# yjh0410/YOLO-Nano

Measured on NVIDIA B200. Metric: images/sec YOLO-Nano-1.0x 416 bs256 fp32-parity e2e (backbone+neck+head+decode+NMS), higher is better.
Workload: dtype f32 (tcgen05 3xTF32 split, fp32 accumulate)

## Files before the change

### yolo_nano_b200/csrc/common.cuh

```cuda
#pragma once
#include <cuda_bf16.h>
#include <cuda_runtime.h>
#include <stdint.h>
#include <limits.h>
#include <stdlib.h>

#include "yolonano_b200.h"

namespace ynb {

constexpr int kNumSMs = 148;

__device__ __forceinline__ float apply_act(float v, int act) {
  if (act == YNB_ACT_RELU) return fmaxf(v, 0.0f);
  if (act == YNB_ACT_LEAKY) return v > 0.0f ? v : 0.1f * v;
  return v;
}

__device__ __forceinline__ float softmax_exp(float d) { return __expf(d); }
__device__ __forceinline__ float class_score(float sum, float obj) { return __fmul_rn(__fdiv_rn(1.0f, sum), obj); }

struct ChanMap {
  int gap_at;
  int gap;
  __host__ __device__ __forceinline__ int slot(int j) const { return j + (j >= gap_at ? gap : 0); }
};
__host__ __device__ inline ChanMap dense_map() { return ChanMap{INT_MAX, 0}; }

// ... 14 lines not shown
  *reinterpret_cast<uint2*>(p) = make_uint2(pack_bf16x2(v.x, v.y), pack_bf16x2(v.z, v.w));
}
__device__ __forceinline__ float to_float(float v) { return v; }
__device__ __forceinline__ float to_float(bf16 v) { return __bfloat162float(v); }

inline int round_up(int v, int m) { return (v + m - 1) / m * m; }
inline int64_t round_up64(int64_t v, int64_t m) { return (v + m - 1) / m * m; }

struct LaunchCounter {
  int64_t n = 0;
};
extern thread_local LaunchCounter* g_counter;

__device__ __forceinline__ void pdl_trigger() { asm volatile("griddepcontrol.launch_dependents;" ::: "memory"); }
__device__ __forceinline__ void pdl_wait() { asm volatile("griddepcontrol.wait;" ::: "memory"); }

inline bool pdl_enabled() {
  static int v = -1;
  if (v < 0) v = getenv("YNB_NO_PDL") ? 0 : 1;
  return v == 1;
}

template <typename... KArgs, typename... Args>
inline cudaError_t launch_pdl(void (*kern)(KArgs...), dim3 grid, dim3 block, size_t smem, cudaStream_t st,
                              Args&&... args) {
  cudaLaunchConfig_t cfg{};
  cfg.gridDim = grid;
  cfg.blockDim = block;
  cfg.dynamicSmemBytes = smem;
  cfg.stream = st;
  cudaLaunchAttribute attr[1];
  attr[0].id = cudaLaunchAttributeProgrammaticStreamSerialization;
  attr[0].val.programmaticStreamSerializationAllowed = 1;
  cfg.attrs = attr;
  cfg.numAttrs = pdl_enabled() ? 1 : 0;
  return cudaLaunchKernelEx(&cfg, kern, static_cast<KArgs>(args)...);
}

#define YNB_COUNT_LAUNCH()                  \
  do {                                      \
    if (::ynb::g_counter) ::ynb::g_counter->n++; \
  } while (0)

}
```

### yolo_nano_b200/csrc/gemm_tc.cuh

```cuda
#pragma once
#include <cuda.h>

#include <cstring>

#include "common.cuh"
#include "ptx_sm100.cuh"

namespace ynb {

constexpr int kTcThreads = 512;
constexpr int kTcSplitWarp0 = 8, kTcProducerWarp = 12, kTcMmaWarp = 13;
constexpr int kTcProducers = 3;
constexpr int kTcBM = 128;
constexpr int kTcBK = 32;
constexpr int kTcAStageBytes = kTcBM * 128;
constexpr int kTcMaxStages = 8;
constexpr int kTcSmemBudget = 232448;
constexpr int kTcMaxMain = 4;

struct TcGemmParams {
  int num_steps;
  int chunks_per_tap;
  int is3x3;
  int mode;
  int bf16_in;
  int out_bf16;
  int num_stages;
  int w_resident;
  int64_t M;
  int64_t num_tiles;
  int H, W, TH, TW, tiles_x, tiles_y;
  int N, Npad;
  int nmain;
  int nacc;
  int merge_corr;
  int ksub;
  int presplit;
  int a2_step;
  int stack_b;
  int acc_stages;
  uint32_t tmem_cols;
  uint32_t a_box_bytes;
  float* out;
  int out_ld, out_off, out_step;
  ChanMap omap;
  const float* bias;
  int act;
  const float* pass;
  int pass_ld;
  int tma_store;
  struct Decode {
// ... 61 lines not shown
  const int box_alo = p.presplit ? 1 : -1;
  const int box_whi = p.w_resident ? -1 : 1 + (p.presplit ? 1 : 0);
  const int box_wlo = (p.w_resident || !split) ? -1 : box_whi + 1;
  const int nboxes = 1 + (box_alo >= 0) + (box_whi >= 0) + (box_wlo >= 0);
  const int nprod = nboxes < kTcProducers ? nboxes : kTcProducers;
  const TcSmemLayout lay = tc_smem_layout(p.Npad, p.num_steps, p.num_stages, p.w_resident != 0, split);
  const uint32_t w_chunk_bytes = lay.w_chunk_bytes;
  const uint32_t a_bytes = kTcAStageBytes * (split ? 2 : 1);
  const uint32_t stage_bytes = lay.stage_bytes;
  const uint32_t w_res_bytes = lay.bias_off - lay.w_res_off;
  float* s_bias = reinterpret_cast<float*>(smem + lay.bias_off);
  uint64_t* bars = reinterpret_cast<uint64_t*>(smem + lay.bar_off);
  uint64_t* full = bars;
  uint64_t* ready = bars + kTcMaxStages;
  uint64_t* empty = bars + 2 * kTcMaxStages;
  uint64_t* tmem_full = bars + 3 * kTcMaxStages;
  uint64_t* tmem_empty = bars + 3 * kTcMaxStages + 2;
  uint64_t* w_full = bars + 3 * kTcMaxStages + 4;
  uint32_t* tmem_ptr = reinterpret_cast<uint32_t*>(bars + 3 * kTcMaxStages + 5);

  const int warp = threadIdx.x >> 5, lane = threadIdx.x & 31;
  pdl_trigger();

  if (warp == kTcProducerWarp && lane == 0) {
    ptx::prefetch_tmap(&tmA);
    if (p.presplit || p.a2_step > 0) ptx::prefetch_tmap(&tmAlo);
    ptx::prefetch_tmap(&tmWhi);
    if (split) ptx::prefetch_tmap(&tmWlo);
    if (p.tma_store) ptx::prefetch_tmap(&tmOut);
    for (int s = 0; s < p.num_stages; ++s) {
      ptx::mbar_init(&full[s], nprod);
      ptx::mbar_init(&ready[s], 4);
      ptx::mbar_init(&empty[s], 1);
    }
    for (int a = 0; a < 2; ++a) {
      ptx::mbar_init(&tmem_full[a], 1);
      ptx::mbar_init(&tmem_empty[a], 4);
    }
    ptx::mbar_init(w_full, 1);
    ptx::fence_barrier_init();
  }
  if (warp == kTcMmaWarp) {
    ptx::tmem_alloc(tmem_ptr, p.tmem_cols);
    ptx::tmem_relinquish();
  }
  if (warp < 4) {
    for (int i = threadIdx.x; i < p.Npad; i += 128) s_bias[i] = i < p.N ? __ldg(p.bias + i) : 0.0f;
  }
  ptx::tc_fence_before_sync();
  __syncthreads();
  ptx::tc_fence_after_sync();
  const uint32_t tmem_base = *tmem_ptr;

  auto stage_a = [&](int s) { return smem + (size_t)s * stage_bytes; };
  auto stage_alo = [&](int s) { return smem + (size_t)s * stage_bytes + kTcAStageBytes; };
  auto w_hi_ptr = [&](int s, int step) {
    return p.w_resident ? smem + lay.w_res_off + (size_t)step * w_chunk_bytes * (split ? 2 : 1)
                        : smem + (size_t)s * stage_bytes + a_bytes;
  };
  auto w_lo_ptr = [&](int s, int step) { return w_hi_ptr(s, step) + w_chunk_bytes; };

  const int acc_cols = p.Npad * p.nacc;
  const uint32_t step_tx = p.a_box_bytes * (p.presplit ? 2 : 1) + (p.w_resident ? 0 : w_chunk_bytes * (split ? 2 : 1));
  const bool splitters_on = split && !p.presplit;

  if (warp == kTcProducerWarp && p.w_resident && ptx::elect_one()) {
    ptx::mbar_arrive_expect_tx(w_full, w_res_bytes);
    for (int st = 0; st < p.num_steps; ++st) {
      ptx::tma_load_2d(w_hi_ptr(0, st), &tmWhi, w_full, st * kchunk, 0);
      if (split) ptx::tma_load_2d(w_lo_ptr(0, st), &tmWlo, w_full, st * kchunk, 0);
    }
  }
  pdl_wait();

  const int prole = warp == kTcProducerWarp ? 0 : (warp == 14 ? 1 : (warp == 15 ? 2 : -1));
  if (prole >= 0) {
    if (prole < nprod && ptx::elect_one()) {
      const bool do_a = 0 % nprod == prole;
      const bool do_alo = box_alo >= 0 && box_alo % nprod == prole;
      const bool do_whi = box_whi >= 0 && box_whi % nprod == prole;
      const bool do_wlo = box_wlo >= 0 && box_wlo % nprod == prole;
      const uint32_t my_tx = (do_a ? p.a_box_bytes : 0u) + (do_alo ? p.a_box_bytes : 0u) +
                             (do_whi ? w_chunk_bytes : 0u) + (do_wlo ? w_chunk_bytes : 0u);
      int s = 0;
      uint32_t ph = 0;
      bool ok = true;
      for (int64_t tile = blockIdx.x; tile < p.num_tiles && ok; tile += gridDim.x) {
        int b = 0, y0 = 0, x0 = 0;
        if (p.is3x3) {
          int per_img = p.tiles_x * p.tiles_y;
          b = (int)(tile / per_img);
          int r = (int)(tile - (int64_t)b * per_img);
          y0 = (r / p.tiles_x) * p.TH;
          x0 = (r % p.tiles_x) * p.TW;
        }
        for (int st = 0; st < p.num_steps; ++st) {
          ok = ptx::mbar_wait(&empty[s], ph ^ 1, p.err_flag, 1);
          if (!ok) break;
          ptx::mbar_arrive_expect_tx(&full[s], my_tx);
          if (p.is3x3) {
            int tap = st / p.chunks_per_tap, kc = st - tap * p.chunks_per_tap;
            int dy = tap / 3, dx = tap - dy * 3;
            if (do_a) ptx::tma_load_4d(stage_a(s), &tmA, &full[s], kc * kchunk, x0 + dx - 1, y0 + dy - 1, b);
            if (do_alo) ptx::tma_load_4d(stage_alo(s), &tmAlo, &full[s], kc * kchunk, x0 + dx - 1, y0 + dy - 1, b);
          } else {
            if (do_a) {
              const bool second = p.a2_step > 0 && st >= p.a2_step;
              ptx::tma_load_2d(stage_a(s), second ? &tmAlo : &tmA, &full[s], (second ? st - p.a2_step : st) * kchunk,
                               (int)(tile * kTcBM));
            }
          }
          if (do_whi) ptx::tma_load_2d(w_hi_ptr(s, st), &tmWhi, &full[s], st * kchunk, 0);
          if (do_wlo) ptx::tma_load_2d(w_lo_ptr(s, st), &tmWlo, &full[s], st * kchunk, 0);
          if (prole == 0) YNB_TRACE(1, tile, st);
          if (++s == p.num_stages) { s = 0; ph ^= 1; }
        }
      }
    }
  } else if (warp == kTcMmaWarp) {
    if (ptx::elect_one()) {
      const uint32_t idesc = ptx::make_idesc(2 , kTcBM, p.Npad);
      const uint32_t idesc2 = ptx::make_idesc(2, kTcBM, 2 * p.Npad);
      const uint32_t idesc_bf = ptx::make_idesc(1 , kTcBM, p.Npad);
      int s = 0;
      uint32_t ph = 0;
      int acc = 0;
      uint32_t acc_ph = 0;
      bool ok = true;
      if (p.w_resident) ok = ptx::mbar_wait(w_full, 0, p.err_flag, 2);
      for (int64_t tile = blockIdx.x; tile < p.num_tiles && ok; tile += gridDim.x) {
        ok = ptx::mbar_wait(&tmem_empty[acc], acc_ph ^ 1, p.err_flag, 3);
        if (!ok) break;
        ptx::tc_fence_after_sync();
        const uint32_t d_tmem = tmem_base + (uint32_t)(acc * acc_cols);
        const uint32_t c_tmem = p.merge_corr ? d_tmem : d_tmem + (uint32_t)(p.nmain * p.Npad);
        int t = 0;
        for (int st = 0; st < p.num_steps; ++st) {
          ok = ptx::mbar_wait(splitters_on ? &ready[s] : &full[s], ph, p.err_flag, 4);
          if (!ok) break;
          ptx::tc_fence_after_sync();
          const uint32_t a_hi = ptx::smem_u32(stage_a(s));
          const uint32_t a_lo = ptx::smem_u32(stage_alo(s));
          const uint32_t b_hi = ptx::smem_u32(w_hi_ptr(s, st));
          const uint32_t b_lo = ptx::smem_u32(w_lo_ptr(s, st));
          const int nk = p.ksub > 0 ? min(kTcBK / 8, p.ksub - st * (kTcBK / 8)) : kTcBK / 8;
          if (p.bf16_in) {
#pragma unroll
            for (int k = 0; k < kTcBK / 8; ++k, ++t) {
              if (k >= nk) break;
              ptx::mma_bf16_ss(d_tmem, ptx::make_sw128_kmajor_desc(a_hi + k * 32), ptx::make_sw128_kmajor_desc(b_hi + k * 32),
                               idesc_bf, t != 0);
            }
          } else if (p.stack_b) {
// ... 1 lines not shown
            for (int k = 0; k < kTcBK / 8; ++k, ++t) {
              if (k >= nk) break;
              const uint64_t db = ptx::make_sw128_kmajor_desc(b_hi + k * 32);
              ptx::mma_tf32_ss(d_tmem, ptx::make_sw128_kmajor_desc(a_hi + k * 32), db, idesc2, t != 0);
              ptx::mma_tf32_ss(c_tmem, ptx::make_sw128_kmajor_desc(a_lo + k * 32), db, idesc, 1);
            }
          } else {
#pragma unroll
            for (int k = 0; k < kTcBK / 8; ++k, ++t) {
              if (k >= nk) break;
              const uint32_t ko = k * 32;
              const uint64_t da = ptx::make_sw128_kmajor_desc(a_hi + ko);
              const uint64_t db = ptx::make_sw128_kmajor_desc(b_hi + ko);
              const int slot = t % p.nmain;
              if (split) {
                ptx::mma_tf32_ss(c_tmem, ptx::make_sw128_kmajor_desc(a_lo + ko), db, idesc, t != 0);
                ptx::mma_tf32_ss(c_tmem, da, ptx::make_sw128_kmajor_desc(b_lo + ko), idesc, 1);
              }
              ptx::mma_tf32_ss(d_tmem + (uint32_t)(slot * p.Npad), da, db, idesc,
                               (split && p.merge_corr) ? 1 : (t >= p.nmain));
            }
          }
          YNB_TRACE(3, tile, st);
          ptx::mma_commit(&empty[s]);
          if (st == p.num_steps - 1) ptx::mma_commit(&tmem_full[acc]);
          if (++s == p.num_stages) { s = 0; ph ^= 1; }
        }
        if (++acc == p.acc_stages) { acc = 0; acc_ph ^= 1; }
      }
    }
  } else if (warp >= kTcSplitWarp0 && warp < kTcSplitWarp0 + 4) {
    if (splitters_on) {
      const int t = threadIdx.x - kTcSplitWarp0 * 32;
      int s = 0;
      uint32_t ph = 0;
      bool ok = true;
      for (int64_t tile = blockIdx.x; tile < p.num_tiles && ok; tile += gridDim.x) {
        for (int st = 0; st < p.num_steps; ++st) {
          ok = ptx::mbar_wait(&full[s], ph, p.err_flag, 5);
          if (!ok) break;
          uint4* a = reinterpret_cast<uint4*>(stage_a(s));
          uint4* lo = reinterpret_cast<uint4*>(stage_alo(s));
#pragma unroll
          for (int i = 0; i < kTcAStageBytes / 16 / 128; ++i) {
            const uint4 v = a[t + i * 128];
            uint4 h, l;
            h.x = rn_tf32_bits(v.x); h.y = rn_tf32_bits(v.y); h.z = rn_tf32_bits(v.z); h.w = rn_tf32_bits(v.w);
            l.x = rn_tf32_bits(__float_as_uint(__uint_as_float(v.x) - __uint_as_float(h.x)));
            l.y = rn_tf32_bits(__float_as_uint(__uint_as_float(v.y) - __uint_as_float(h.y)));
            l.z = rn_tf32_bits(__float_as_uint(__uint_as_float(v.z) - __uint_as_float(h.z)));
            l.w = rn_tf32_bits(__float_as_uint(__uint_as_float(v.w) - __uint_as_float(h.w)));
            a[t + i * 128] = h;
            lo[t + i * 128] = l;
          }
          ptx::fence_proxy_async_smem();
          __syncwarp();
          if (lane == 0) ptx::mbar_arrive(&ready[s]);
          if (t == 0) YNB_TRACE(2, tile, st);
          if (++s == p.num_stages) { s = 0; ph ^= 1; }
        }
      }
    }
  } else if (warp < 8) {
    const int group = warp >> 2;
    const int q = warp & 3;
    const int row = q * 32 + lane;
    const bool vec = p.out_step == 1 && p.omap.gap == 0;
    const float slope = p.act == YNB_ACT_RELU ? 0.0f : (p.act == YNB_ACT_LEAKY ? 0.1f : 1.0f);
    uint8_t* sbox = smem + lay.stg_off + warp * 4096;
    const int sw = lane & 7;
    const int nloc = (int64_t)blockIdx.x < p.num_tiles
                         ? (int)((p.num_tiles - blockIdx.x + gridDim.x - 1) / gridDim.x) : 0;
    const bool share_last = kDecC == 0;
    const int col_split = min(p.Npad, ((p.Npad / 2 + 31) / 32) * 32);
    bool ok = true;
    for (int lt = 0; lt < nloc && ok; ++lt) {
      const int64_t tile = blockIdx.x + (int64_t)lt * gridDim.x;
      const int acc = p.acc_stages == 2 ? (lt & 1) : 0;
      const bool shared = share_last && lt == nloc - 1 && col_split < p.Npad;
      if (!shared && group != acc) {
        if (p.acc_stages == 1 && share_last) ok = ptx::mbar_wait(&tmem_full[0], (uint32_t)(lt & 1), p.err_flag, 7);
        continue;
      }
      const int col_begin = shared && group == 1 ? col_split : 0;
      const int col_end = shared && group == 0 ? col_split : p.Npad;
      const uint32_t acc_ph = (uint32_t)((lt / p.acc_stages) & 1);
      int64_t m;
      bool valid;
      if (p.is3x3) {
        int per_img = p.tiles_x * p.tiles_y;
        int b = (int)(tile / per_img);
        int r = (int)(tile - (int64_t)b * per_img);
        int y = (r / p.tiles_x) * p.TH + row / p.TW;
        int x = (r % p.tiles_x) * p.TW + row % p.TW;
        valid = row < p.TH * p.TW && y < p.H && x < p.W;
        m = ((int64_t)b * p.H + y) * p.W + x;
      } else {
        m = tile * kTcBM + row;
        valid = m < p.M;
      }
// ... 227 lines not shown
            }
          } else {
            const int64_t off = valid ? m * p.out_ld : -1;
#pragma unroll 8
            for (int r = 0; r < 32; ++r) {
              const int64_t offr = __shfl_sync(0xffffffffu, off, r);
              if (col_ok && offr >= 0) {
                if (p.out_bf16) out_bf[offr + col] = __float2bfloat16_rn(staged(r, lane));
                else p.out[offr + col] = staged(r, lane);
              }
            }
          }
        }
        __syncwarp();
      }
      if (lane == 0 && q == 0) YNB_TRACE(5, tile, group);
    }
    __syncwarp();
    if (p.tma_store && ptx::elect_one()) ptx::bulk_wait<0>();
  }

  ptx::tc_fence_before_sync();
  __syncthreads();
  if (warp == kTcMmaWarp) {
    ptx::tc_fence_after_sync();
    ptx::tmem_dealloc(tmem_base, p.tmem_cols);
  }
}

typedef CUresult (*PFN_encodeTiled)(CUtensorMap*, CUtensorMapDataType, cuuint32_t, void*, const cuuint64_t*,
                                    const cuuint64_t*, const cuuint32_t*, const cuuint32_t*,
                                    CUtensorMapInterleave, CUtensorMapSwizzle, CUtensorMapL2promotion,
                                    CUtensorMapFloatOOBfill);

inline PFN_encodeTiled get_encode_tiled() {
  static PFN_encodeTiled fn = nullptr;
  if (!fn) {
    void* p = nullptr;
    cudaDriverEntryPointQueryResult qres;
    if (cudaGetDriverEntryPoint("cuTensorMapEncodeTiled", &p, cudaEnableDefault, &qres) == cudaSuccess &&
        qres == cudaDriverEntryPointSuccess)
      fn = reinterpret_cast<PFN_encodeTiled>(p);
  }
  return fn;
}

// ... 37 lines not shown
             CU_TENSOR_MAP_INTERLEAVE_NONE, CU_TENSOR_MAP_SWIZZLE_NONE, CU_TENSOR_MAP_L2_PROMOTION_L2_128B,
             CU_TENSOR_MAP_FLOAT_OOB_FILL_NONE) == CUDA_SUCCESS;
}

inline bool make_tmap_out(CUtensorMap* m, void* base, uint64_t cols, uint64_t rows, uint64_t ld, bool bf16 = false) {
  PFN_encodeTiled enc = get_encode_tiled();
  if (!enc) return false;
  const uint64_t es = bf16 ? 2 : 4;
  cuuint64_t dims[2] = {cols, rows};
  cuuint64_t strides[1] = {ld * es};
  cuuint32_t box[2] = {32, 32};
  cuuint32_t estr[2] = {1, 1};
  return enc(m, bf16 ? CU_TENSOR_MAP_DATA_TYPE_BFLOAT16 : CU_TENSOR_MAP_DATA_TYPE_FLOAT32, 2, base, dims, strides, box,
             estr, CU_TENSOR_MAP_INTERLEAVE_NONE, bf16 ? CU_TENSOR_MAP_SWIZZLE_NONE : CU_TENSOR_MAP_SWIZZLE_128B,
             CU_TENSOR_MAP_L2_PROMOTION_NONE, CU_TENSOR_MAP_FLOAT_OOB_FILL_NONE) == CUDA_SUCCESS;
}

struct TcWeights {
  float* hi = nullptr;
  float* lo = nullptr;
  bf16* bw = nullptr;
  int N = 0, Npad = 0, Kpad = 0;
  CUtensorMap tm_hi, tm_lo;
};

inline void split_tf32_host(float v, float* hi, float* lo) {
  uint32_t u;
  memcpy(&u, &v, 4);
  uint32_t h = rn_tf32_bits(u);
  float hf;
  memcpy(&hf, &h, 4);
  float l = v - hf;
  uint32_t lu;
  memcpy(&lu, &l, 4);
  lu = rn_tf32_bits(lu);
  memcpy(lo, &lu, 4);
  *hi = hf;
}

struct TcGemmLaunch {
  CUtensorMap tmA;
  CUtensorMap tmOut;
  const TcWeights* w = nullptr;
  CUtensorMap tmAlo;
  TcGemmParams p;
  uint32_t smem = 0;
  unsigned grid = 0;
// ... 34 lines not shown
  static const bool no_stack = getenv("YNB_TC_NO_STACK") != nullptr;
  p.stack_b = (split && !no_stack && p.nmain == 1 && p.nacc == 2 && 2 * p.Npad <= 256 && (2 * p.Npad) % 16 == 0) ? 1 : 0;
}

inline bool tc_plan_smem(TcGemmLaunch& L) {
  TcGemmParams& p = L.p;
  const bool split = p.mode == YNB_GEMM_TC_3XTF32;
  for (int resident = 1; resident >= 0; --resident) {
    for (int stages = kTcMaxStages; stages >= 2; --stages) {
      if (stages > p.num_steps * 4 && stages > 2) continue;
      TcSmemLayout lay = tc_smem_layout(p.Npad, p.num_steps, stages, resident != 0, split);
      static const bool res2 = getenv("YNB_TC_RES2") != nullptr;
      if (lay.total <= (uint32_t)kTcSmemBudget && (resident == 0 || stages >= 3 || p.num_steps <= 2 || res2)) {
        p.num_stages = stages;
        p.w_resident = resident;
        L.smem = lay.total;
        return true;
      }
    }
  }
  return false;
}

inline cudaError_t launch_tc_gemm(const TcGemmLaunch& L, cudaStream_t st) {
  using KernelT = void (*)(CUtensorMap, CUtensorMap, CUtensorMap, CUtensorMap, CUtensorMap, TcGemmParams);
  static const KernelT kernels[4] = {tc_gemm_kernel<false, 0>, tc_gemm_kernel<true, 0>, tc_gemm_kernel<false, 80>,
                                     tc_gemm_kernel<false, 20>};
  static bool attr_set = false;
  if (!attr_set) {
    for (KernelT k : kernels) {
      cudaError_t e = cudaFuncSetAttribute(k, cudaFuncAttributeMaxDynamicSharedMemorySize, kTcSmemBudget);
      if (e != cudaSuccess) return e;
    }
    attr_set = true;
  }
  const CUtensorMap& tmo = L.p.tma_store ? L.tmOut : L.tmA;
  KernelT kern = L.dec_classes == 80 ? kernels[2] : (L.dec_classes == 20 ? kernels[3] : kernels[L.p.pass != nullptr ? 1 : 0]);
  const CUtensorMap& tmalo = (L.p.presplit || L.p.a2_step > 0) ? L.tmAlo : L.tmA;
  cudaError_t r = launch_pdl(kern, dim3(L.grid), dim3(kTcThreads), (size_t)L.smem, st, L.tmA, tmalo, L.w->tm_hi,
                             L.w->tm_lo, tmo, L.p);
  YNB_COUNT_LAUNCH();
  return r;
}

inline void tc_pick_tile(int H, int W, int* TH, int* TW) {
  double best = -1;
  for (int tw = 4; tw <= 64 && tw <= W + 3; ++tw) {
    int th = 128 / tw;
    if (th < 1) continue;
    if (th > H) th = H;
    double eff = (double)H * W / ((double)((W + tw - 1) / tw) * ((H + th - 1) / th) * 128.0);
    if (eff > best + 1e-9) { best = eff; *TH = th; *TW = tw; }
  }
}

}
```

### yolo_nano_b200/csrc/ptx_sm100.cuh

```cuda
#pragma once
#include <cuda.h>
#include <cuda_runtime.h>
#include <stdint.h>

namespace ynb {
namespace ptx {

__device__ __forceinline__ uint32_t smem_u32(const void* p) {
  return (uint32_t)__cvta_generic_to_shared(p);
}

__device__ __forceinline__ void mbar_init(uint64_t* bar, uint32_t count) {
  asm volatile("mbarrier.init.shared::cta.b64 [%0], %1;" ::"r"(smem_u32(bar)), "r"(count));
}
__device__ __forceinline__ void fence_barrier_init() {
  asm volatile("fence.mbarrier_init.release.cluster;" ::: "memory");
}
__device__ __forceinline__ void mbar_arrive(uint64_t* bar) {
  asm volatile("mbarrier.arrive.shared::cta.b64 _, [%0];" ::"r"(smem_u32(bar)) : "memory");
}
__device__ __forceinline__ void mbar_arrive_expect_tx(uint64_t* bar, uint32_t bytes) {
  asm volatile("mbarrier.arrive.expect_tx.shared::cta.b64 _, [%0], %1;" ::"r"(smem_u32(bar)), "r"(bytes)
               : "memory");
}
// ... 36 lines not shown
}
__device__ __forceinline__ void tc_fence_after_sync() {
  asm volatile("tcgen05.fence::after_thread_sync;" ::: "memory");
}

__device__ __forceinline__ void prefetch_tmap(const CUtensorMap* m) {
  asm volatile("prefetch.tensormap [%0];" ::"l"(reinterpret_cast<uint64_t>(m)) : "memory");
}
__device__ __forceinline__ void tma_load_2d(void* smem_dst, const CUtensorMap* m, uint64_t* bar, int c0, int c1) {
  asm volatile(
      "cp.async.bulk.tensor.2d.shared::cluster.global.mbarrier::complete_tx::bytes [%0], [%1, {%3, %4}], [%2];"
      ::"r"(smem_u32(smem_dst)), "l"(reinterpret_cast<uint64_t>(m)), "r"(smem_u32(bar)), "r"(c0), "r"(c1)
      : "memory");
}
__device__ __forceinline__ void tma_load_4d(void* smem_dst, const CUtensorMap* m, uint64_t* bar, int c0, int c1,
                                            int c2, int c3) {
  asm volatile(
      "cp.async.bulk.tensor.4d.shared::cluster.global.mbarrier::complete_tx::bytes [%0], [%1, {%3, %4, %5, %6}], [%2];"
      ::"r"(smem_u32(smem_dst)), "l"(reinterpret_cast<uint64_t>(m)), "r"(smem_u32(bar)), "r"(c0), "r"(c1),
      "r"(c2), "r"(c3)
      : "memory");
}

__device__ __forceinline__ void tma_prefetch_4d(const CUtensorMap* m, int c0, int c1, int c2, int c3) {
  asm volatile("cp.async.bulk.prefetch.tensor.4d.L2.global.tile [%0, {%1, %2, %3, %4}];"
               ::"l"(reinterpret_cast<uint64_t>(m)), "r"(c0), "r"(c1), "r"(c2), "r"(c3)
               : "memory");
}

__device__ __forceinline__ void cp_async_16(void* smem_dst, const void* gsrc, uint32_t src_bytes) {
  asm volatile("cp.async.cg.shared.global [%0], [%1], 16, %2;" ::"r"(smem_u32(smem_dst)), "l"(gsrc), "r"(src_bytes)
               : "memory");
}
__device__ __forceinline__ void cp_async_commit() { asm volatile("cp.async.commit_group;" ::: "memory"); }
__device__ __forceinline__ void cp_async_wait_all() { asm volatile("cp.async.wait_group 0;" ::: "memory"); }

__device__ __forceinline__ void tma_store_2d(const CUtensorMap* m, const void* smem_src, int c0, int c1) {
  asm volatile("cp.async.bulk.tensor.2d.global.shared::cta.bulk_group [%0, {%2, %3}], [%1];"
               ::"l"(reinterpret_cast<uint64_t>(m)), "r"(smem_u32(smem_src)), "r"(c0), "r"(c1)
               : "memory");
}
__device__ __forceinline__ void tma_store_4d(const CUtensorMap* m, const void* smem_src, int c0, int c1, int c2, int c3) {
  asm volatile("cp.async.bulk.tensor.4d.global.shared::cta.bulk_group [%0, {%2, %3, %4, %5}], [%1];"
               ::"l"(reinterpret_cast<uint64_t>(m)), "r"(smem_u32(smem_src)), "r"(c0), "r"(c1), "r"(c2), "r"(c3)
               : "memory");
}
// ... 34 lines not shown
}
__device__ __forceinline__ void mma_tf32_ss(uint32_t tmem_d, uint64_t adesc, uint64_t bdesc, uint32_t idesc,
                                            uint32_t accumulate) {
  asm volatile(
      "{\n\t.reg .pred p;\n\t"
      "setp.ne.b32 p, %4, 0;\n\t"
      "tcgen05.mma.cta_group::1.kind::tf32 [%0], %1, %2, %3, p;\n\t}"
      ::"r"(tmem_d), "l"(adesc), "l"(bdesc), "r"(idesc), "r"(accumulate)
      : "memory");
}
__device__ __forceinline__ void mma_bf16_ss(uint32_t tmem_d, uint64_t adesc, uint64_t bdesc, uint32_t idesc,
                                            uint32_t accumulate) {
  asm volatile(
      "{\n\t.reg .pred p;\n\t"
      "setp.ne.b32 p, %4, 0;\n\t"
      "tcgen05.mma.cta_group::1.kind::f16 [%0], %1, %2, %3, p;\n\t}"
      ::"r"(tmem_d), "l"(adesc), "l"(bdesc), "r"(idesc), "r"(accumulate)
      : "memory");
}
__device__ __forceinline__ void mma_commit(uint64_t* bar) {
  asm volatile("tcgen05.commit.cta_group::1.mbarrier::arrive::one.shared::cluster.b64 [%0];" ::"r"(smem_u32(bar))
               : "memory");
}

__device__ __forceinline__ void tmem_ld_32x32(uint32_t taddr, uint32_t (&r)[32]) {
  asm volatile(
      "tcgen05.ld.sync.aligned.32x32b.x32.b32 "
      "{%0, %1, %2, %3, %4, %5, %6, %7, %8, %9, %10, %11, %12, %13, %14, %15, "
      "%16, %17, %18, %19, %20, %21, %22, %23, %24, %25, %26, %27, %28, %29, %30, %31}, [%32];"
      : "=r"(r[0]), "=r"(r[1]), "=r"(r[2]), "=r"(r[3]), "=r"(r[4]), "=r"(r[5]), "=r"(r[6]), "=r"(r[7]),
        "=r"(r[8]), "=r"(r[9]), "=r"(r[10]), "=r"(r[11]), "=r"(r[12]), "=r"(r[13]), "=r"(r[14]), "=r"(r[15]),
        "=r"(r[16]), "=r"(r[17]), "=r"(r[18]), "=r"(r[19]), "=r"(r[20]), "=r"(r[21]), "=r"(r[22]), "=r"(r[23]),
        "=r"(r[24]), "=r"(r[25]), "=r"(r[26]), "=r"(r[27]), "=r"(r[28]), "=r"(r[29]), "=r"(r[30]), "=r"(r[31])
      : "r"(taddr)
      : "memory");
}
__device__ __forceinline__ void tmem_ld_32x16(uint32_t taddr, uint32_t (&r)[16]) {
  asm volatile(
      "tcgen05.ld.sync.aligned.32x32b.x16.b32 "
      "{%0, %1, %2, %3, %4, %5, %6, %7, %8, %9, %10, %11, %12, %13, %14, %15}, [%16];"
      : "=r"(r[0]), "=r"(r[1]), "=r"(r[2]), "=r"(r[3]), "=r"(r[4]), "=r"(r[5]), "=r"(r[6]), "=r"(r[7]),
        "=r"(r[8]), "=r"(r[9]), "=r"(r[10]), "=r"(r[11]), "=r"(r[12]), "=r"(r[13]), "=r"(r[14]), "=r"(r[15])
      : "r"(taddr)
      : "memory");
}
__device__ __forceinline__ void tmem_ld_wait() {
// ... 29 lines not shown
```

### yolo_nano_b200/csrc/ynb_api.cu

```cuda
#include <cuda.h>
#include <cuda_runtime.h>

#include <cmath>
#include <cstdio>
#include <cstdlib>
#include <cstring>
#include <deque>
#include <functional>
#include <map>
#include <memory>
#include <string>
#include <tuple>
#include <vector>

#include "yolonano_b200.h"

#include "common.cuh"
#include "decode_nms.cuh"
#include "nms_grid.cuh"
#include "gemm_ffma.cuh"
#include "gemm_tc.cuh"
#include "unit_tc.cuh"
#include "kernels_basic.cuh"
#include "train_ops.cuh"
// ... 215 lines not shown
    const int kin = ktot / taps, kin_pad = round_up(kin, 64);
    t.Kpad = taps * kin_pad;
    std::vector<bf16> bw((size_t)t.Npad * t.Kpad, __float2bfloat16(0.0f));
    for (int r = 0; r < n; ++r)
      for (int tp = 0; tp < taps; ++tp)
        for (int k = 0; k < kin; ++k)
          bw[(size_t)r * t.Kpad + (size_t)tp * kin_pad + k] = __float2bfloat16_rn(w[(size_t)r * ktot + (size_t)tp * kin + k]);
    CUDA_TRY(e, cudaMalloc(&t.bw, bw.size() * 2));
    CUDA_TRY(e, cudaMemcpy(t.bw, bw.data(), bw.size() * 2, cudaMemcpyHostToDevice));
    if (!make_tmap_2d(&t.tm_hi, t.bw, t.Kpad, t.Npad, t.Kpad, t.Npad, true))
      return fail(e, YNB_ERR_CUDA, "cuTensorMapEncodeTiled failed for weights of " + name);
    t.tm_lo = t.tm_hi;
    return YNB_OK;
  }
  t.Kpad = round_up(ktot, kTcBK);
  std::vector<float> hi((size_t)t.Npad * t.Kpad, 0.f), lo((size_t)t.Npad * t.Kpad, 0.f);
  for (int r = 0; r < n; ++r)
    for (int k = 0; k < ktot; ++k)
      split_tf32_host(w[(size_t)r * ktot + k], &hi[(size_t)r * t.Kpad + k], &lo[(size_t)r * t.Kpad + k]);
  CUDA_TRY(e, cudaMalloc(&t.hi, hi.size() * 4));
  CUDA_TRY(e, cudaMalloc(&t.lo, lo.size() * 4));
  CUDA_TRY(e, cudaMemcpy(t.hi, hi.data(), hi.size() * 4, cudaMemcpyHostToDevice));
  CUDA_TRY(e, cudaMemcpy(t.lo, lo.data(), lo.size() * 4, cudaMemcpyHostToDevice));
  if (!make_tmap_2d(&t.tm_hi, t.hi, t.Kpad, t.Npad, t.Kpad, t.Npad) ||
      !make_tmap_2d(&t.tm_lo, t.lo, t.Kpad, t.Npad, t.Kpad, t.Npad))
    return fail(e, YNB_ERR_CUDA, "cuTensorMapEncodeTiled failed for weights of " + name);
  return YNB_OK;
}

int pack_cat(ynb_engine* e, int si) {
  const bool bf = is_bf16(e);
  const std::string bk = "backbone.stage" + std::to_string(si + 2) + ".0.";
  const int i1 = e->index.at(bk + "branch1.2"), i2 = e->index.at(bk + "branch2.5");
  const ConvSpec& c1 = e->table[i1];
  const ConvSpec& c2 = e->table[i2];
  const PackedConv& p1 = e->convs[i1];
  const PackedConv& p2 = e->convs[i2];
  const InLayout il1 = in_layout(c1, bf), il2 = in_layout(c2, bf);
  const StageLayout sl = stage_layout(bf, si);
  const int ch = bf ? 64 : kTcBK;
  const int k1p = round_up(il1.ktot, ch), k2p = round_up(il2.ktot, ch), ktot = k1p + k2p;
  const int h = c1.cout;
  std::vector<float> w((size_t)sl.ld * ktot, 0.f), b((size_t)sl.ld, 0.f);
  for (int i = 0; i < h; ++i) {
    const int r1 = sl.map.slot(2 * i), r2 = sl.map.slot(2 * i + 1);
    for (int k = 0; k < c1.cin; ++k) w[(size_t)r1 * ktot + il1.map.slot(k)] = p1.w_host[(size_t)i * c1.cin + k];
    for (int k = 0; k < c2.cin; ++k) w[(size_t)r2 * ktot + k1p + il2.map.slot(k)] = p2.w_host[(size_t)i * c2.cin + k];
    b[r1] = p1.b_host[i];
// ... 275 lines not shown
    p.N = pc.n; p.Npad = pc.tc.Npad;
    tc_plan_tmem(p, name.size() > 2 && name.compare(0, 8, "head_det") == 0 && name.compare(name.size() - 2, 2, ".4") == 0);
    p.a_box_bytes = kTcAStageBytes;
    p.out = out.p; p.out_ld = out.ld; p.out_off = out_off; p.out_step = out_step; p.omap = out.map;
    p.bias = pc.b_dev; p.act = c.act;
    p.pass = pass ? pass->p : nullptr; p.pass_ld = pass ? pass->ld : 0;
    p.err_flag = e->d_err;
    if (dec) {
      p.dec = *dec;
      L.dec_classes = e->cfg.num_classes;
    }
    const int oal = 16 / out.es;
    p.tma_store = (!dec && !pass && out_step == 1 && out.map.gap == 0 && out_off % oal == 0 && out.ld % oal == 0) ? 1 : 0;
    if (p.tma_store && !make_tmap_out(&L.tmOut, out.at(out_off), (uint64_t)round_up(pc.n, oal), (uint64_t)M,
                                      (uint64_t)out.ld, out.es == 2)) {
      error = "cuTensorMapEncodeTiled failed for output of " + name;
      return;
    }
    if (!make_tmap_2d(&L.tmA, in.at(in_off), (uint64_t)pc.ktot, (uint64_t)M, (uint64_t)in.ld, kTcBM, bf)) {
      error = "cuTensorMapEncodeTiled failed for input of " + name;
      return;
    }
    if (!tc_plan_smem(L)) { error = "no smem configuration for " + name; return; }
    L.grid = (unsigned)std::min<int64_t>(p.num_tiles, kNumSMs);
    const TcGemmLaunch* Lp = &L;
    const double obytes = dec ? abytes - (double)out.es * M * c.cout + 24.0 * M * 3 : abytes;
    Op op{dec ? name + "+decode" : name, dec ? "pw_decode_tcgen05" : "pw_tcgen05", obytes, aflops,
          [=](cudaStream_t st) { return launch_tc_gemm(*Lp, st); }};
    op.join = join;
    ops().push_back(op);
  }

  bool catpw(int si, const std::string& unit, const Tensor& b1dw, const Tensor& mid2, const Tensor& out) {
    static const bool off = getenv("YNB_NO_CAT_GEMM") != nullptr;
    if (off || e->cfg.gemm_mode == YNB_GEMM_FP32_FFMA || e->cat[si].empty()) return false;
    const bool bf = is_bf16(e);
    const int64_t M = (int64_t)B * out.H * out.W;
    const ConvSpec& c1 = spec(unit + "branch1.2");
    const ConvSpec& c2 = spec(unit + "branch2.5");
    for (size_t pi = 0; pi < e->cat[si].size(); ++pi) {
      const ynb_engine::CatConv& cc = e->cat[si][pi];
      tc->emplace_back();
      TcGemmLaunch& L = tc->back();
      L.w = &cc.pc.tc;
      TcGemmParams& p = L.p;
      memset(&p, 0, sizeof(p));
      p.mode = e->cfg.gemm_mode;
// ... 1 lines not shown
      p.out_bf16 = out.es == 2 ? 1 : 0;
      const int ch = bf ? 64 : kTcBK;
      p.num_steps = cc.pc.tc.Kpad / ch;
      p.chunks_per_tap = p.num_steps;
      p.a2_step = cc.k1p / ch;
      p.ksub = 0;
      p.M = M;
      p.num_tiles = (M + kTcBM - 1) / kTcBM;
      p.N = cc.pc.n; p.Npad = cc.pc.tc.Npad;
      tc_plan_tmem(p);
      p.a_box_bytes = kTcAStageBytes;
      p.out = out.p; p.out_ld = out.ld; p.out_off = cc.n0; p.out_step = 1; p.omap = dense_map();
      p.bias = cc.pc.b_dev; p.act = c1.act;
      p.err_flag = e->d_err;
      p.tma_store = 1;
      const int oal = 16 / out.es;
      if (!make_tmap_out(&L.tmOut, out.at(cc.n0), (uint64_t)round_up(cc.pc.n, oal), (uint64_t)M, (uint64_t)out.ld, out.es == 2) ||
          !make_tmap_2d(&L.tmA, b1dw.p, (uint64_t)b1dw.ld, (uint64_t)M, (uint64_t)b1dw.ld, kTcBM, bf) ||
          !make_tmap_2d(&L.tmAlo, mid2.p, (uint64_t)mid2.ld, (uint64_t)M, (uint64_t)mid2.ld, kTcBM, bf)) {
        error = "cuTensorMapEncodeTiled failed for the merged stride-2 conv of " + unit;
        return true;
      }
      if (!tc_plan_smem(L)) { error = "no smem configuration for the merged stride-2 conv of " + unit; return true; }
      L.grid = (unsigned)std::min<int64_t>(p.num_tiles, kNumSMs);
      const TcGemmLaunch* Lp = &L;
      const double frac = (double)cc.pc.n / out.ld;
      const double bytes = (double)b1dw.es * M * (c1.cin + c2.cin) + (double)out.es * M * 2.0 * c1.cout * frac +
                           (bf ? 2.0 : 4.0) * (c1.cin + c2.cin) * c1.cout;
      const double flops = 2.0 * M * (c1.cin + c2.cin) * c1.cout * frac;
      ops().push_back({unit + "branch1.2|branch2.5" + (e->cat[si].size() > 1 ? "." + std::to_string(pi) : ""), "pw_tcgen05", bytes,
                       flops, [=](cudaStream_t st) { return launch_tc_gemm(*Lp, st); }});
    }
    return true;
  }

  bool dwpw(const std::string& dw_name, const std::string& pw_name, const Tensor& in, const Tensor& out,
            const Tensor* pass) {
    static const bool off = getenv("YNB_NO_FUSED_DWPW") != nullptr;
    if (off || e->cfg.gemm_mode == YNB_GEMM_FP32_FFMA) return false;
    const PackedConv& dc = conv(dw_name);
    const PackedConv& pc = conv(pw_name);
    const ConvSpec& ds = spec(dw_name);
    const ConvSpec& ps = spec(pw_name);
    if (ds.stride != 1 || dc.n != pc.ktot) return false;
    dp->emplace_back();
    DwPwLaunch& L = dp->back();
    DwPwParams& p = L.p;
// ... 938 lines not shown
  int rc = YNB_OK;
  TcGemmLaunch L;
  L.w = &t;
  TcGemmParams& p = L.p;
  memset(&p, 0, sizeof(p));
  p.mode = mode; p.num_steps = t.Kpad / kTcBK; p.chunks_per_tap = p.num_steps; p.ksub = (cin + 7) / 8;
  p.M = pixels; p.num_tiles = (pixels + kTcBM - 1) / kTcBM; p.N = cout; p.Npad = t.Npad;
  tc_plan_tmem(p);
  p.a_box_bytes = kTcAStageBytes;
  p.out = out; p.out_ld = out_ld; p.out_off = out_off; p.out_step = out_step; p.omap = dense_map();
  p.bias = b_dev; p.act = act; p.err_flag = d_err;
  long long* d_trace = nullptr;
  const int trace_cap = 8 * 64 * 32;
  const bool want_trace = getenv("YNB_TC_TRACE") != nullptr;
  if (want_trace) {
    UNIT_TRY(cudaMalloc(&d_trace, (1 + 4 * trace_cap) * 8));
    UNIT_TRY(cudaMemset(d_trace, 0, (1 + 4 * trace_cap) * 8));
    p.trace = d_trace; p.trace_cap = trace_cap;
  }
  p.tma_store = (out_step == 1 && out_off % 4 == 0 && getenv("YNB_TC_NO_TMA_STORE") == nullptr) ? 1 : 0;
  if (getenv("YNB_TC_PASS") != nullptr && cin >= cout && out_ld >= 2 * cout) {
    p.pass = in; p.pass_ld = in_ld; p.tma_store = 0; p.out_off = 1; p.out_step = 2;
  }
  if (!make_tmap_2d(&t.tm_hi, t.hi, t.Kpad, t.Npad, t.Kpad, t.Npad) ||
      !make_tmap_2d(&t.tm_lo, t.lo, t.Kpad, t.Npad, t.Kpad, t.Npad) ||
      (p.tma_store && !make_tmap_out(&L.tmOut, out + out_off, (uint64_t)round_up(cout, 4), (uint64_t)pixels,
                                     (uint64_t)out_ld)) ||
      !make_tmap_2d(&L.tmA, in + in_off, cin, pixels, in_ld, kTcBM) || !tc_plan_smem(L)) {
    rc = fail(nullptr, YNB_ERR_CUDA, "ynb_pwconv_tc: tensor map / smem planning failed");
  } else {
    L.grid = (unsigned)std::min<int64_t>(p.num_tiles, kNumSMs);
    cudaError_t r = launch_tc_gemm(L, st);
    if (r == cudaSuccess) r = cudaStreamSynchronize(st);
    int flag = 0;
    if (r == cudaSuccess) r = cudaMemcpy(&flag, d_err, 4, cudaMemcpyDeviceToHost);
    if (r != cudaSuccess) rc = fail(nullptr, YNB_ERR_CUDA, std::string("ynb_pwconv_tc: ") + cudaGetErrorString(r));
    else if (flag) rc = fail(nullptr, YNB_ERR_CUDA, "ynb_pwconv_tc: mbarrier timeout code " + std::to_string(flag));
    if (want_trace && r == cudaSuccess) {
      std::vector<long long> h(1 + 4 * trace_cap);
      cudaMemcpy(h.data(), d_trace, h.size() * 8, cudaMemcpyDeviceToHost);
      int n = 0;
      for (int i = 0; i < trace_cap; ++i) n += h[4 + 4 * i] != 0;
      fprintf(stderr, "YNB_TC_TRACE stages=%d resident=%d nmain=%d acc_stages=%d steps=%d grid=%u events=%d\n",
              p.num_stages, p.w_resident, p.nmain, p.acc_stages, p.num_steps, L.grid, n);
      for (int i = 0; i < trace_cap; ++i)
        if (h[4 + 4 * i] != 0)
          fprintf(stderr, "TRACE %lld %lld %lld %lld\n", h[1 + 4 * i], h[2 + 4 * i], h[3 + 4 * i], h[4 + 4 * i]);
    }
  }
  if (d_trace) cudaFree(d_trace);
  cudaFree(t.hi); cudaFree(t.lo); cudaFree(d_err);
  return rc;
}

YNB_EXPORT int ynb_dwpw_tc(const float* in, int32_t in_ld, const float* dw_w, const float* dw_b, int32_t dw_act,
                           const float* pw_w, const float* pw_b, int32_t act, float* out, int32_t out_ld,
                           const float* pass, int32_t pass_ld, int32_t batch, int32_t h, int32_t w_, int32_t channels,
                           int32_t cout, int32_t mode, void* stream) {
  const bool bfm = mode == YNB_GEMM_TC_BF16;
  const int al = bfm ? 8 : 4;
  if (!in || !dw_w || !dw_b || !pw_w || !pw_b || !out || channels % al || in_ld % al || out_ld % al || cout > (bfm ? 240 : 128) ||
      cout < 1 || batch < 1 || h < 1 || w_ < 1 ||
      (mode != YNB_GEMM_TC_3XTF32 && mode != YNB_GEMM_TC_TF32 && mode != YNB_GEMM_TC_BF16) ||
      (pass && (out_ld < 2 * cout || pass_ld < cout || pass_ld % 4 || ((uintptr_t)pass & 15u))) || (!pass && out_ld < cout) ||
      ((uintptr_t)out & 15u))
    return fail(nullptr, YNB_ERR_INVALID, "ynb_dwpw_tc: bad arguments");
  cudaStream_t st = (cudaStream_t)stream;
// ... 801 lines not shown
```

Before: 35010.

## Multicast streamed GEMM weights across 2-CTA clusters in tcgen05 pointwise kernel

When weights are not SMEM-resident and the conv is 1x1 fp32, the TC GEMM is launched with 2-CTA clusters. Each CTA loads half of the weight rows per k-step and multicasts them to both CTAs, so each CTA issues half the weight TMA traffic. Empty barriers now take arrivals from both CTAs through multicast tcgen05.commit, tiles are assigned in cluster-paired groups, and a drain loop plus cluster syncs keep either CTA from exiting early. In exchange, the two CTAs of a cluster run in lockstep, and grid size is limited by cluster occupancy.

```diff
diff --git a/yolo_nano_b200/csrc/common.cuh b/yolo_nano_b200/csrc/common.cuh
--- a/yolo_nano_b200/csrc/common.cuh
+++ b/yolo_nano_b200/csrc/common.cuh
@@ -4,6 +4,8 @@
 #include <stdint.h>
 #include <limits.h>
 #include <stdlib.h>
+
+#include <utility>
 
 #include "yolonano_b200.h"
 
@@ -64,19 +66,34 @@
 }
 
 template <typename... KArgs, typename... Args>
-inline cudaError_t launch_pdl(void (*kern)(KArgs...), dim3 grid, dim3 block, size_t smem, cudaStream_t st,
-                              Args&&... args) {
+inline cudaError_t launch_pdl_cluster(void (*kern)(KArgs...), dim3 grid, dim3 block, size_t smem, cudaStream_t st,
+                                      unsigned cluster, Args&&... args) {
   cudaLaunchConfig_t cfg{};
   cfg.gridDim = grid;
   cfg.blockDim = block;
   cfg.dynamicSmemBytes = smem;
   cfg.stream = st;
-  cudaLaunchAttribute attr[1];
-  attr[0].id = cudaLaunchAttributeProgrammaticStreamSerialization;
-  attr[0].val.programmaticStreamSerializationAllowed = 1;
+  cudaLaunchAttribute attr[2];
+  unsigned n = 0;
+  if (pdl_enabled()) {
+    attr[n].id = cudaLaunchAttributeProgrammaticStreamSerialization;
+    attr[n++].val.programmaticStreamSerializationAllowed = 1;
+  }
+  if (cluster > 1) {
+    attr[n].id = cudaLaunchAttributeClusterDimension;
+    attr[n].val.clusterDim.x = cluster;
+    attr[n].val.clusterDim.y = 1;
+    attr[n++].val.clusterDim.z = 1;
+  }
   cfg.attrs = attr;
-  cfg.numAttrs = pdl_enabled() ? 1 : 0;
+  cfg.numAttrs = n;
   return cudaLaunchKernelEx(&cfg, kern, static_cast<KArgs>(args)...);
+}
+
+template <typename... KArgs, typename... Args>
+inline cudaError_t launch_pdl(void (*kern)(KArgs...), dim3 grid, dim3 block, size_t smem, cudaStream_t st,
+                              Args&&... args) {
+  return launch_pdl_cluster(kern, grid, block, smem, st, 1u, std::forward<Args>(args)...);
 }
 
 #define YNB_COUNT_LAUNCH()                  \
diff --git a/yolo_nano_b200/csrc/gemm_tc.cuh b/yolo_nano_b200/csrc/gemm_tc.cuh
--- a/yolo_nano_b200/csrc/gemm_tc.cuh
+++ b/yolo_nano_b200/csrc/gemm_tc.cuh
@@ -1,6 +1,7 @@
 #pragma once
 #include <cuda.h>
 
+#include <algorithm>
 #include <cstring>
 
 #include "common.cuh"
@@ -27,6 +28,7 @@
   int out_bf16;
   int num_stages;
   int w_resident;
+  int cluster;
   int64_t M;
   int64_t num_tiles;
   int H, W, TH, TW, tiles_x, tiles_y;
@@ -134,6 +136,12 @@
   const int warp = threadIdx.x >> 5, lane = threadIdx.x & 31;
   pdl_trigger();
 
+  const int ccta = p.cluster > 1 ? p.cluster : 1;
+  const int crank = (int)(blockIdx.x % ccta);
+  const int64_t grp0 = blockIdx.x / ccta, grp_step = gridDim.x / ccta;
+  const int64_t ngroups = (p.num_tiles + ccta - 1) / ccta;
+  const uint16_t cmask = (uint16_t)((1u << ccta) - 1);
+
   if (warp == kTcProducerWarp && lane == 0) {
     ptx::prefetch_tmap(&tmA);
     if (p.presplit || p.a2_step > 0) ptx::prefetch_tmap(&tmAlo);
@@ -143,7 +151,7 @@
     for (int s = 0; s < p.num_stages; ++s) {
       ptx::mbar_init(&full[s], nprod);
       ptx::mbar_init(&ready[s], 4);
-      ptx::mbar_init(&empty[s], 1);
+      ptx::mbar_init(&empty[s], ccta);
     }
     for (int a = 0; a < 2; ++a) {
       ptx::mbar_init(&tmem_full[a], 1);
@@ -161,6 +169,7 @@
   }
   ptx::tc_fence_before_sync();
   __syncthreads();
+  if (ccta > 1) ptx::cluster_sync();
   ptx::tc_fence_after_sync();
   const uint32_t tmem_base = *tmem_ptr;
 
@@ -194,10 +203,14 @@
       const bool do_wlo = box_wlo >= 0 && box_wlo % nprod == prole;
       const uint32_t my_tx = (do_a ? p.a_box_bytes : 0u) + (do_alo ? p.a_box_bytes : 0u) +
                              (do_whi ? w_chunk_bytes : 0u) + (do_wlo ? w_chunk_bytes : 0u);
+      const int w_rows = p.Npad / ccta;
+      const int w_row0 = crank * w_rows;
+      const uint32_t w_off = (uint32_t)w_row0 * 128u;
       int s = 0;
       uint32_t ph = 0;
       bool ok = true;
-      for (int64_t tile = blockIdx.x; tile < p.num_tiles && ok; tile += gridDim.x) {
+      for (int64_t g = grp0; g < ngroups && ok; g += grp_step) {
+        const int64_t tile = g * ccta + crank;
         int b = 0, y0 = 0, x0 = 0;
         if (p.is3x3) {
           int per_img = p.tiles_x * p.tiles_y;
@@ -222,9 +235,20 @@
                                (int)(tile * kTcBM));
             }
           }
-          if (do_whi) ptx::tma_load_2d(w_hi_ptr(s, st), &tmWhi, &full[s], st * kchunk, 0);
-          if (do_wlo) ptx::tma_load_2d(w_lo_ptr(s, st), &tmWlo, &full[s], st * kchunk, 0);
+          if (ccta > 1) {
+            if (do_whi) ptx::tma_load_2d_mcast(w_hi_ptr(s, st) + w_off, &tmWhi, &full[s], st * kchunk, w_row0, cmask);
+            if (do_wlo) ptx::tma_load_2d_mcast(w_lo_ptr(s, st) + w_off, &tmWlo, &full[s], st * kchunk, w_row0, cmask);
+          } else {
+            if (do_whi) ptx::tma_load_2d(w_hi_ptr(s, st), &tmWhi, &full[s], st * kchunk, 0);
+            if (do_wlo) ptx::tma_load_2d(w_lo_ptr(s, st), &tmWlo, &full[s], st * kchunk, 0);
+          }
           if (prole == 0) YNB_TRACE(1, tile, st);
+          if (++s == p.num_stages) { s = 0; ph ^= 1; }
+        }
+      }
+      if (ccta > 1 && prole == 0) {
+        for (int i = 0; i < p.num_stages && ok; ++i) {
+          ok = ptx::mbar_wait(&empty[s], ph ^ 1, p.err_flag, 8);
           if (++s == p.num_stages) { s = 0; ph ^= 1; }
         }
       }
@@ -240,7 +264,8 @@
       uint32_t acc_ph = 0;
       bool ok = true;
       if (p.w_resident) ok = ptx::mbar_wait(w_full, 0, p.err_flag, 2);
-      for (int64_t tile = blockIdx.x; tile < p.num_tiles && ok; tile += gridDim.x) {
+      for (int64_t g = grp0; g < ngroups && ok; g += grp_step) {
+        const int64_t tile = g * ccta + crank;
         ok = ptx::mbar_wait(&tmem_empty[acc], acc_ph ^ 1, p.err_flag, 3);
         if (!ok) break;
         ptx::tc_fence_after_sync();
@@ -288,7 +313,8 @@
             }
           }
           YNB_TRACE(3, tile, st);
-          ptx::mma_commit(&empty[s]);
+          if (ccta > 1) ptx::mma_commit_mcast(&empty[s], cmask);
+          else ptx::mma_commit(&empty[s]);
           if (st == p.num_steps - 1) ptx::mma_commit(&tmem_full[acc]);
           if (++s == p.num_stages) { s = 0; ph ^= 1; }
         }
@@ -301,7 +327,8 @@
       int s = 0;
       uint32_t ph = 0;
       bool ok = true;
-      for (int64_t tile = blockIdx.x; tile < p.num_tiles && ok; tile += gridDim.x) {
+      for (int64_t g = grp0; g < ngroups && ok; g += grp_step) {
+        const int64_t tile = g * ccta + crank;
         for (int st = 0; st < p.num_steps; ++st) {
           ok = ptx::mbar_wait(&full[s], ph, p.err_flag, 5);
           if (!ok) break;
@@ -335,13 +362,12 @@
     const float slope = p.act == YNB_ACT_RELU ? 0.0f : (p.act == YNB_ACT_LEAKY ? 0.1f : 1.0f);
     uint8_t* sbox = smem + lay.stg_off + warp * 4096;
     const int sw = lane & 7;
-    const int nloc = (int64_t)blockIdx.x < p.num_tiles
-                         ? (int)((p.num_tiles - blockIdx.x + gridDim.x - 1) / gridDim.x) : 0;
+    const int nloc = grp0 < ngroups ? (int)((ngroups - grp0 + grp_step - 1) / grp_step) : 0;
     const bool share_last = kDecC == 0;
     const int col_split = min(p.Npad, ((p.Npad / 2 + 31) / 32) * 32);
     bool ok = true;
     for (int lt = 0; lt < nloc && ok; ++lt) {
-      const int64_t tile = blockIdx.x + (int64_t)lt * gridDim.x;
+      const int64_t tile = (grp0 + (int64_t)lt * grp_step) * ccta + crank;
       const int acc = p.acc_stages == 2 ? (lt & 1) : 0;
       const bool shared = share_last && lt == nloc - 1 && col_split < p.Npad;
       if (!shared && group != acc) {
@@ -615,6 +641,7 @@
 
   ptx::tc_fence_before_sync();
   __syncthreads();
+  if (ccta > 1) ptx::cluster_sync();
   if (warp == kTcMmaWarp) {
     ptx::tc_fence_after_sync();
     ptx::tmem_dealloc(tmem_base, p.tmem_cols);
@@ -698,7 +725,23 @@
   bf16* bw = nullptr;
   int N = 0, Npad = 0, Kpad = 0;
   CUtensorMap tm_hi, tm_lo;
+  bool has_half = false;
+  CUtensorMap tm_hi_half, tm_lo_half;
 };
+
+inline bool make_tc_weight_tmaps(TcWeights& t) {
+  t.has_half = false;
+  if (!make_tmap_2d(&t.tm_hi, t.hi, t.Kpad, t.Npad, t.Kpad, t.Npad) ||
+      !make_tmap_2d(&t.tm_lo, t.lo, t.Kpad, t.Npad, t.Kpad, t.Npad))
+    return false;
+  if (t.Npad % 16 == 0) {
+    if (!make_tmap_2d(&t.tm_hi_half, t.hi, t.Kpad, t.Npad, t.Kpad, t.Npad / 2) ||
+        !make_tmap_2d(&t.tm_lo_half, t.lo, t.Kpad, t.Npad, t.Kpad, t.Npad / 2))
+      return false;
+    t.has_half = true;
+  }
+  return true;
+}
 
 inline void split_tf32_host(float v, float* hi, float* lo) {
   uint32_t u;
@@ -779,23 +822,57 @@
   return false;
 }
 
-inline cudaError_t launch_tc_gemm(const TcGemmLaunch& L, cudaStream_t st) {
-  using KernelT = void (*)(CUtensorMap, CUtensorMap, CUtensorMap, CUtensorMap, CUtensorMap, TcGemmParams);
-  static const KernelT kernels[4] = {tc_gemm_kernel<false, 0>, tc_gemm_kernel<true, 0>, tc_gemm_kernel<false, 80>,
-                                     tc_gemm_kernel<false, 20>};
+using TcKernelT = void (*)(CUtensorMap, CUtensorMap, CUtensorMap, CUtensorMap, CUtensorMap, TcGemmParams);
+
+inline TcKernelT tc_kernel_for(const TcGemmLaunch& L) {
+  static const TcKernelT kernels[4] = {tc_gemm_kernel<false, 0>, tc_gemm_kernel<true, 0>, tc_gemm_kernel<false, 80>,
+                                       tc_gemm_kernel<false, 20>};
   static bool attr_set = false;
   if (!attr_set) {
-    for (KernelT k : kernels) {
-      cudaError_t e = cudaFuncSetAttribute(k, cudaFuncAttributeMaxDynamicSharedMemorySize, kTcSmemBudget);
-      if (e != cudaSuccess) return e;
-    }
+    for (TcKernelT k : kernels)
+      if (cudaFuncSetAttribute(k, cudaFuncAttributeMaxDynamicSharedMemorySize, kTcSmemBudget) != cudaSuccess) return nullptr;
     attr_set = true;
   }
+  return L.dec_classes == 80 ? kernels[2] : (L.dec_classes == 20 ? kernels[3] : kernels[L.p.pass != nullptr ? 1 : 0]);
+}
+
+inline void tc_plan_grid(TcGemmLaunch& L) {
+  TcGemmParams& p = L.p;
+  p.cluster = 1;
+  L.grid = (unsigned)std::min<int64_t>(p.num_tiles, kNumSMs);
+  const char* env = getenv("YNB_TC_MCAST");
+  if ((env && env[0] == '0') || p.w_resident || p.is3x3 || p.bf16_in || !L.w->has_half || p.num_tiles < 2) return;
+  TcKernelT kern = tc_kernel_for(L);
+  if (!kern) return;
+  cudaLaunchConfig_t cfg{};
+  cudaLaunchAttribute attr[1];
+  attr[0].id = cudaLaunchAttributeClusterDimension;
+  attr[0].val.clusterDim.x = 2;
+  attr[0].val.clusterDim.y = 1;
+  attr[0].val.clusterDim.z = 1;
+  cfg.gridDim = dim3(kNumSMs);
+  cfg.blockDim = dim3(kTcThreads);
+  cfg.dynamicSmemBytes = L.smem;
+  cfg.attrs = attr;
+  cfg.numAttrs = 1;
+  int nclusters = 0;
+  if (cudaOccupancyMaxActiveClusters(&nclusters, kern, &cfg) != cudaSuccess || nclusters < 1) {
+    cudaGetLastError();
+    return;
+  }
+  p.cluster = 2;
+  L.grid = 2u * (unsigned)std::min<int64_t>((p.num_tiles + 1) / 2, std::min(nclusters, kNumSMs / 2));
+}
+
+inline cudaError_t launch_tc_gemm(const TcGemmLaunch& L, cudaStream_t st) {
+  TcKernelT kern = tc_kernel_for(L);
+  if (!kern) return cudaErrorInvalidValue;
   const CUtensorMap& tmo = L.p.tma_store ? L.tmOut : L.tmA;
-  KernelT kern = L.dec_classes == 80 ? kernels[2] : (L.dec_classes == 20 ? kernels[3] : kernels[L.p.pass != nullptr ? 1 : 0]);
   const CUtensorMap& tmalo = (L.p.presplit || L.p.a2_step > 0) ? L.tmAlo : L.tmA;
-  cudaError_t r = launch_pdl(kern, dim3(L.grid), dim3(kTcThreads), (size_t)L.smem, st, L.tmA, tmalo, L.w->tm_hi,
-                             L.w->tm_lo, tmo, L.p);
+  const bool half = L.p.cluster == 2;
+  cudaError_t r = launch_pdl_cluster(kern, dim3(L.grid), dim3(kTcThreads), (size_t)L.smem, st, half ? 2u : 1u, L.tmA,
+                                     tmalo, half ? L.w->tm_hi_half : L.w->tm_hi, half ? L.w->tm_lo_half : L.w->tm_lo,
+                                     tmo, L.p);
   YNB_COUNT_LAUNCH();
   return r;
 }
diff --git a/yolo_nano_b200/csrc/ptx_sm100.cuh b/yolo_nano_b200/csrc/ptx_sm100.cuh
--- a/yolo_nano_b200/csrc/ptx_sm100.cuh
+++ b/yolo_nano_b200/csrc/ptx_sm100.cuh
@@ -82,6 +82,19 @@
       : "memory");
 }
 
+__device__ __forceinline__ void tma_load_2d_mcast(void* smem_dst, const CUtensorMap* m, uint64_t* bar, int c0, int c1,
+                                                  uint16_t cta_mask) {
+  asm volatile(
+      "cp.async.bulk.tensor.2d.shared::cluster.global.mbarrier::complete_tx::bytes.multicast::cluster"
+      " [%0], [%1, {%4, %5}], [%2], %3;"
+      ::"r"(smem_u32(smem_dst)), "l"(reinterpret_cast<uint64_t>(m)), "r"(smem_u32(bar)), "h"(cta_mask), "r"(c0), "r"(c1)
+      : "memory");
+}
+
+__device__ __forceinline__ void cluster_sync() {
+  asm volatile("barrier.cluster.arrive.release.aligned;\n\tbarrier.cluster.wait.acquire.aligned;" ::: "memory");
+}
+
 __device__ __forceinline__ void tma_prefetch_4d(const CUtensorMap* m, int c0, int c1, int c2, int c3) {
   asm volatile("cp.async.bulk.prefetch.tensor.4d.L2.global.tile [%0, {%1, %2, %3, %4}];"
                ::"l"(reinterpret_cast<uint64_t>(m)), "r"(c0), "r"(c1), "r"(c2), "r"(c3)
@@ -162,6 +175,12 @@
   asm volatile("tcgen05.commit.cta_group::1.mbarrier::arrive::one.shared::cluster.b64 [%0];" ::"r"(smem_u32(bar))
                : "memory");
 }
+__device__ __forceinline__ void mma_commit_mcast(uint64_t* bar, uint16_t cta_mask) {
+  asm volatile(
+      "tcgen05.commit.cta_group::1.mbarrier::arrive::one.shared::cluster.multicast::cluster.b64 [%0], %1;"
+      ::"r"(smem_u32(bar)), "h"(cta_mask)
+      : "memory");
+}
 
 __device__ __forceinline__ void tmem_ld_32x32(uint32_t taddr, uint32_t (&r)[32]) {
   asm volatile(
diff --git a/yolo_nano_b200/csrc/ynb_api.cu b/yolo_nano_b200/csrc/ynb_api.cu
--- a/yolo_nano_b200/csrc/ynb_api.cu
+++ b/yolo_nano_b200/csrc/ynb_api.cu
@@ -261,8 +261,7 @@
   CUDA_TRY(e, cudaMalloc(&t.lo, lo.size() * 4));
   CUDA_TRY(e, cudaMemcpy(t.hi, hi.data(), hi.size() * 4, cudaMemcpyHostToDevice));
   CUDA_TRY(e, cudaMemcpy(t.lo, lo.data(), lo.size() * 4, cudaMemcpyHostToDevice));
-  if (!make_tmap_2d(&t.tm_hi, t.hi, t.Kpad, t.Npad, t.Kpad, t.Npad) ||
-      !make_tmap_2d(&t.tm_lo, t.lo, t.Kpad, t.Npad, t.Kpad, t.Npad))
+  if (!make_tc_weight_tmaps(t))
     return fail(e, YNB_ERR_CUDA, "cuTensorMapEncodeTiled failed for weights of " + name);
   return YNB_OK;
 }
@@ -584,7 +583,7 @@
       return;
     }
     if (!tc_plan_smem(L)) { error = "no smem configuration for " + name; return; }
-    L.grid = (unsigned)std::min<int64_t>(p.num_tiles, kNumSMs);
+    tc_plan_grid(L);
     const TcGemmLaunch* Lp = &L;
     const double obytes = dec ? abytes - (double)out.es * M * c.cout + 24.0 * M * 3 : abytes;
     Op op{dec ? name + "+decode" : name, dec ? "pw_decode_tcgen05" : "pw_tcgen05", obytes, aflops,
@@ -632,7 +631,7 @@
         return true;
       }
       if (!tc_plan_smem(L)) { error = "no smem configuration for the merged stride-2 conv of " + unit; return true; }
-      L.grid = (unsigned)std::min<int64_t>(p.num_tiles, kNumSMs);
+      tc_plan_grid(L);
       const TcGemmLaunch* Lp = &L;
       const double frac = (double)cc.pc.n / out.ld;
       const double bytes = (double)b1dw.es * M * (c1.cin + c2.cin) + (double)out.es * M * 2.0 * c1.cout * frac +
@@ -1617,14 +1616,13 @@
   if (getenv("YNB_TC_PASS") != nullptr && cin >= cout && out_ld >= 2 * cout) {
     p.pass = in; p.pass_ld = in_ld; p.tma_store = 0; p.out_off = 1; p.out_step = 2;
   }
-  if (!make_tmap_2d(&t.tm_hi, t.hi, t.Kpad, t.Npad, t.Kpad, t.Npad) ||
-      !make_tmap_2d(&t.tm_lo, t.lo, t.Kpad, t.Npad, t.Kpad, t.Npad) ||
+  if (!make_tc_weight_tmaps(t) ||
       (p.tma_store && !make_tmap_out(&L.tmOut, out + out_off, (uint64_t)round_up(cout, 4), (uint64_t)pixels,
                                      (uint64_t)out_ld)) ||
       !make_tmap_2d(&L.tmA, in + in_off, cin, pixels, in_ld, kTcBM) || !tc_plan_smem(L)) {
     rc = fail(nullptr, YNB_ERR_CUDA, "ynb_pwconv_tc: tensor map / smem planning failed");
   } else {
-    L.grid = (unsigned)std::min<int64_t>(p.num_tiles, kNumSMs);
+    tc_plan_grid(L);
     cudaError_t r = launch_tc_gemm(L, st);
     if (r == cudaSuccess) r = cudaStreamSynchronize(st);
     int flag = 0;
@@ -1636,8 +1634,8 @@
       cudaMemcpy(h.data(), d_trace, h.size() * 8, cudaMemcpyDeviceToHost);
       int n = 0;
       for (int i = 0; i < trace_cap; ++i) n += h[4 + 4 * i] != 0;
-      fprintf(stderr, "YNB_TC_TRACE stages=%d resident=%d nmain=%d acc_stages=%d steps=%d grid=%u events=%d\n",
-              p.num_stages, p.w_resident, p.nmain, p.acc_stages, p.num_steps, L.grid, n);
+      fprintf(stderr, "YNB_TC_TRACE stages=%d resident=%d nmain=%d acc_stages=%d steps=%d grid=%u cluster=%d events=%d\n",
+              p.num_stages, p.w_resident, p.nmain, p.acc_stages, p.num_steps, L.grid, p.cluster, n);
       for (int i = 0; i < trace_cap; ++i)
         if (h[4 + 4 * i] != 0)
           fprintf(stderr, "TRACE %lld %lld %lld %lld\n", h[1 + 4 * i], h[2 + 4 * i], h[3 + 4 * i], h[4 + 4 * i]);
```

After: 34660 (median of 6 runs). 0.99x the previous value.
